# One-2-3-45/One-2-3-45

Hardware: AMD Instinct MI355X
Metric: rays/sec + mesh-extract wall-clock per scene (8x256^2 views, 128^3 vol) (higher is better)
Workload: dtype f32 (matrix products as 3 f16 MFMAs on split operands, fp32 accumulate); 1 GPU; BASELINE config 2: 1 scene/GPU/step (a different seeded scene every step), 8 views 256x256, 128^3 volume, 262144 rays (64+64 samples), mesh grid 256^3; whole scene pass per step; views=8, volume=128, rays=262144, mesh_res=256, parallelism=scenes x1, precision=f16x3

## Files before the change

### one-2-3-45_amd/csrc/color_net.h

```cpp
#pragma once
#include "common.h"
#include "geom_math.h"
#include "split_f16.h"

namespace o2345 {

#define MFMA32(a, b, c) __builtin_amdgcn_mfma_f32_32x32x2f32((a), (b), (c), 0, 0, 0)

constexpr int CM_A_RD0 = 0;
constexpr int CM_A_RD1 = CM_A_RD0 + 1 * 2 * 64;
constexpr int CM_A_B0 = CM_A_RD1 + 2 * 8 * 64;
constexpr int CM_A_B1 = CM_A_B0 + 2 * 32 * 64;
constexpr int CM_A_V0 = CM_A_B1 + 32 * 64;
constexpr int CM_A_V1 = CM_A_V0 + 16 * 64;
constexpr int CM_A_V20 = CM_A_V1 + 16 * 64;
constexpr int CM_A_R0 = CM_A_V20 + 16 * 64;
constexpr int CM_A_R1 = CM_A_R0 + 19 * 64;
constexpr int CM_BIAS0 = CM_A_R1 + 8 * 64;
constexpr int CM_B_RD0 = CM_BIAS0, CM_B_RD1 = CM_B_RD0 + 32, CM_B_B0 = CM_B_RD1 + 64, CM_B_B1 = CM_B_B0 + 64,
              CM_B_V0 = CM_B_B1 + 32, CM_B_V1 = CM_B_V0 + 32, CM_B_V20 = CM_B_V1 + 32, CM_B_R0 = CM_B_V20 + 32,
              CM_B_R1 = CM_B_R0 + 32, CM_V_V1X = CM_B_R1 + 32, CM_V_V21 = CM_V_V1X + 32, CM_V_R2 = CM_V_V21 + 32;
constexpr int CM_W_S = CM_V_R2 + 32;
constexpr int CM_S = CM_W_S + 144 * 64;
constexpr int CM_TOTAL = CM_S + 4;
constexpr int CX_A_RD0 = 0;
constexpr int CX_A_RD1 = CX_A_RD0 + 1 * 1 * 512;
constexpr int CX_A_B0 = CX_A_RD1 + 2 * 1 * 512;
constexpr int CX_A_B1 = CX_A_B0 + 2 * 4 * 512;
constexpr int CX_A_V0 = CX_A_B1 + 4 * 512;
constexpr int CX_A_V1 = CX_A_V0 + 2 * 512;
constexpr int CX_A_V20 = CX_A_V1 + 2 * 512;
constexpr int CX_A_R0 = CX_A_V20 + 2 * 512;
constexpr int CX_A_R1 = CX_A_R0 + 3 * 512;
constexpr int CX_A_END = CX_A_R1 + 1 * 512;
constexpr int CX_TOTAL = CX_A_END + (CM_TOTAL - CM_BIAS0);
constexpr int CM_A_S = CM_TOTAL;
constexpr int CM_TOTAL2 = CM_A_S + 2 * 72 * 64;
constexpr int CX_A_S = CX_TOTAL;
constexpr int CX_TOTAL2 = CX_A_S + 2 * 9 * 512;

struct ColorMArgs {
    const float* blob;
    const float* vol_cl; const float* maskvol; int D;
    const float* cmaps; const float* proj; const float* cam_pos; int V, H, W_img;
    const float* pts; const int* index; const int* n_dev; long long n;
    const float* query_cam; const float* normals;
    float* out_rgb; uint8_t* out_nviews;
    const float* f_geo;
    const float* f_rgb;
    const float* f_rdiff;
    const float* f_mask;
    unsigned long long* stats;
    int sched;
};

inline int color_sched_mode() { return knobs().color_sched; }
#if defined(__HIPCC__)
__device__ __forceinline__ void set_wave_prio(int p) {
    switch (p) {
        case 0: __builtin_amdgcn_s_setprio(0); break;
        case 1: __builtin_amdgcn_s_setprio(1); break;
        case 2: __builtin_amdgcn_s_setprio(2); break;
        default: __builtin_amdgcn_s_setprio(3); break;
    }
}
#endif

constexpr float LOG2E = 1.44269504088896340736f, LN2 = 0.69314718055994530942f;
__device__ __forceinline__ float celu(float y) {
    const float t = __builtin_amdgcn_fmed3f(__builtin_amdgcn_exp2f(y), 0.f, 1.f);
    return fmaxf(y, fmaf(t, LOG2E, -LOG2E));
}
typedef float f32x2 __attribute__((ext_vector_type(2)));
__device__ __forceinline__ f32x2 celu2(float y0, float y1) {
    f32x2 t;
    t[0] = __builtin_amdgcn_fmed3f(__builtin_amdgcn_exp2f(y0), 0.f, 1.f);
    t[1] = __builtin_amdgcn_fmed3f(__builtin_amdgcn_exp2f(y1), 0.f, 1.f);
    const f32x2 e = __builtin_elementwise_fma(t, f32x2{LOG2E, LOG2E}, f32x2{-LOG2E, -LOG2E});
    return f32x2{fmaxf(y0, e[0]), fmaxf(y1, e[1])};
}
__device__ __forceinline__ float crcp(float x) { return __builtin_amdgcn_rcpf(x); }
__device__ __forceinline__ float csigm(float z) { return crcp(1.f + __builtin_amdgcn_exp2f(-z)); }

template <int NB, int NST, int N>
__device__ __forceinline__ void cm_run(f32x16 (&acc)[NB], const float* A , int step0, const float (&b)[N]) {
    float cur[NB], nxt[NB];
#pragma unroll
    for (int nb = 0; nb < NB; ++nb) cur[nb] = A[(nb * NST + step0) * 64];
#pragma unroll
    for (int r = 0; r < N; ++r) {
        if (r + 1 < N) {
#pragma unroll
            for (int nb = 0; nb < NB; ++nb) nxt[nb] = A[(nb * NST + step0 + r + 1) * 64];
        }
#pragma unroll
        for (int nb = 0; nb < NB; ++nb) acc[nb] = MFMA32(cur[nb], b[r], acc[nb]);
#pragma unroll
        for (int nb = 0; nb < NB; ++nb) cur[nb] = nxt[nb];
        __builtin_amdgcn_sched_barrier(0);
    }
}

template <int NB, int N>
__device__ __forceinline__ void cx_run(f32x16 (&acc)[NB], const float4* A , const float (&b)[N], float m1) {
    constexpr int NS = (N + 7) / 8;
#pragma unroll
    for (int s = 0; s < NS; ++s) {
        const Split8 sp = split8(b, 8 * s, m1);
        h16x8 ahi[NB], alo[NB];
#pragma unroll
        for (int nb = 0; nb < NB; ++nb) {
            ahi[nb] = __builtin_bit_cast(h16x8, A[((nb * NS + s) * 2 + 0) * 64]);
            alo[nb] = __builtin_bit_cast(h16x8, A[((nb * NS + s) * 2 + 1) * 64]);
        }
#pragma unroll
        for (int nb = 0; nb < NB; ++nb) acc[nb] = MFMA_F16(alo[nb], sp.hi, acc[nb]);
#pragma unroll
        for (int nb = 0; nb < NB; ++nb) acc[nb] = MFMA_F16(ahi[nb], sp.lo, acc[nb]);
#pragma unroll
        for (int nb = 0; nb < NB; ++nb) acc[nb] = MFMA_F16(ahi[nb], sp.hi, acc[nb]);
        __builtin_amdgcn_sched_barrier(0);
    }
}
template <int NB, int N>
__device__ __forceinline__ void cx_run_from(f32x16 (&acc)[NB], const f32x16 (&init)[NB], const float4* A, const float (&b)[N], float m1) {
    constexpr int NS = (N + 7) / 8;
#pragma unroll
    for (int s = 0; s < NS; ++s) {
        const Split8 sp = split8(b, 8 * s, m1);
        h16x8 ahi[NB], alo[NB];
#pragma unroll
        for (int nb = 0; nb < NB; ++nb) {
            ahi[nb] = __builtin_bit_cast(h16x8, A[((nb * NS + s) * 2 + 0) * 64]);
            alo[nb] = __builtin_bit_cast(h16x8, A[((nb * NS + s) * 2 + 1) * 64]);
        }
#pragma unroll
        for (int nb = 0; nb < NB; ++nb) acc[nb] = MFMA_F16(alo[nb], sp.hi, s == 0 ? init[nb] : acc[nb]);
#pragma unroll
        for (int nb = 0; nb < NB; ++nb) acc[nb] = MFMA_F16(ahi[nb], sp.lo, acc[nb]);
#pragma unroll
        for (int nb = 0; nb < NB; ++nb) acc[nb] = MFMA_F16(ahi[nb], sp.hi, acc[nb]);
        __builtin_amdgcn_sched_barrier(0);
    }
}
template <bool X3, int NB, int N>
__device__ __forceinline__ void cm_layer(f32x16 (&acc)[NB], const float* lds, int lane, int off32, int offx, const float (&b)[N], float m1) {
    if constexpr (X3) cx_run<NB, N>(acc, reinterpret_cast<const float4*>(lds + offx) + lane, b, m1);
    else cm_run<NB, N, N>(acc, lds + lane + off32, 0, b);
}

template <int NB>
__device__ __forceinline__ void cm_bias(f32x16 (&acc)[NB], const float* bias, int h) {
#pragma unroll
    for (int nb = 0; nb < NB; ++nb) {
        const float4* p = reinterpret_cast<const float4*>(bias + (nb * 2 + h) * 16);
#pragma unroll
        for (int q = 0; q < 4; ++q) {
            const float4 t = p[q];
            acc[nb][4 * q] = t.x; acc[nb][4 * q + 1] = t.y; acc[nb][4 * q + 2] = t.z; acc[nb][4 * q + 3] = t.w;
        }
    }
}

template <int CTRL>
__device__ __forceinline__ float dpp_mov(float v) {
    return __builtin_bit_cast(float, __builtin_amdgcn_update_dpp(0, __builtin_bit_cast(int, v), CTRL, 0xf, 0xf, true));
}
#define O2345_GROUP_REDUCE(NAME, OP)                                                   \
    template <int G>                                                                   \
    __device__ __forceinline__ float NAME(float v) {                                   \
        v = OP(v, dpp_mov<0xB1>(v));                          \
        v = OP(v, dpp_mov<0x4E>(v));                          \
        if (G >= 8) v = OP(v, dpp_mov<0x141>(v));             \
        if (G >= 16) v = OP(v, dpp_mov<0x140>(v));            \
        if (G >= 32) v = OP(v, __shfl_xor(v, 16));                                     \
        return v;                                                                      \
    }
__device__ __forceinline__ float op_add(float a, float b) { return a + b; }
O2345_GROUP_REDUCE(gsum, op_add)
O2345_GROUP_REDUCE(gmin, fminf)
O2345_GROUP_REDUCE(gmax, fmaxf)
#undef O2345_GROUP_REDUCE

__device__ __forceinline__ void cm_project(const float* __restrict__ P, float x, float y, float z, int H, int W, float& gx, float& gy) {
    const float X = P[0] * x + P[1] * y + P[2] * z + P[3];
    const float Y = P[4] * x + P[5] * y + P[6] * z + P[7];
    const float Z = fmaxf(P[8] * x + P[9] * y + P[10] * z + P[11], 1e-3f);
    const float rz = crcp(Z), rw = crcp((float)(W - 1)), rh = crcp((float)(H - 1));
    auto div = [](float a_, float b_, float r_) { const float q = a_ * r_; return fmaf(fmaf(-b_, q, a_), r_, q); };
    gx = div(2.f * div(X, Z, rz), (float)(W - 1), rw) - 1.f;
    gy = div(2.f * div(Y, Z, rz), (float)(H - 1), rh) - 1.f;
    if (gx > 1.f || gx < -1.f) gx = 2.f;
    if (gy > 1.f || gy < -1.f) gy = 2.f;
}


#if defined(__HIPCC__)
struct ViewGeom {
    float rd[4];
    float e;
    float m;
    float gx, gy;
};

__device__ __forceinline__ ViewGeom view_geom(const ColorMArgs& a, int v, float px, float py, float pz, float qx, float qy, float qz,
                                              bool gvalid, float s_abs) {
    ViewGeom g;
    cm_project(a.proj + 12 * v, px, py, pz, a.H, a.W_img, g.gx, g.gy);
    g.m = (gvalid && fabsf(g.gx) < 1.f && fabsf(g.gy) < 1.f) ? 1.f : 0.f;
    const float sx = a.cam_pos[3 * v] - px, sy = a.cam_pos[3 * v + 1] - py, sz = a.cam_pos[3 * v + 2] - pz;
    const float rsn = crcp(sqrtf(sx * sx + sy * sy + sz * sz) + 1e-6f);
    const float ux = sx * rsn, uy = sy * rsn, uz = sz * rsn;
    const float dx = qx - ux, dy = qy - uy, dz = qz - uz;
    const float rdn = crcp(fmaxf(sqrtf(dx * dx + dy * dy + dz * dz), 1e-6f));
    g.rd[0] = dx * rdn; g.rd[1] = dy * rdn; g.rd[2] = dz * rdn;
    g.rd[3] = qx * ux + qy * uy + qz * uz;
    g.e = __builtin_amdgcn_exp2f(s_abs * (g.rd[3] - 1.f));
    return g;
}

#endif

int project_features_launch(const float* vol_cl, const float* maskvol, int D, const float* cmaps, const float* proj, const float* cam_pos, int V, int H, int W,
                            const float* pts, long long n, const float* query_cam, const float* normals, float* geo, float* rgb_feat, float* rdiff, float* mask,
                            void* stream);
int color_feats_launch(int x3, const float* blob, const float* geo, const float* rgb_feat, const float* ray_diff, const float* mask, int V, long long n,
                       float* out_rgb, uint8_t* out_nviews, void* stream);
int color_pts_launch(int x3, const float* blob, const float* vol_cl, const float* maskvol, int D, const float* cmaps, const float* proj,
                     const float* cam_pos, int V, int H, int W, const float* pts, const int32_t* index, const int32_t* n_dev, long long n,
                     const float* query_cam, const float* normals, float* out_rgb, uint8_t* out_nviews, unsigned long long* stats_dev, void* stream);

}
```

### one-2-3-45_amd/csrc/color_pts.hip

```cpp
#include "color_net.h"

namespace o2345 {

__device__ __forceinline__ void gather_now(const ColorMArgs& a, int h, int v, const ViewGeom& g, float (&rf)[32]) {
#pragma unroll
    for (int c = 0; c < 32; ++c) rf[c] = 0.f;
    const Taps2D tp = bilinear_taps(g.gx, g.gy, a.H, a.W_img);
    const float4* img = reinterpret_cast<const float4*>(a.cmaps + (size_t)v * a.H * a.W_img * 64) + 8 * h;
#pragma unroll
    for (int k = 0; k < 4; ++k)
        if (tp.w[k] != 0.f) {
            const float4* px4 = img + (size_t)tp.idx[k] * 16;
            const float wk = tp.w[k] * LOG2E;
#pragma unroll
            for (int q = 0; q < 8; ++q) {
                const float4 t = px4[q];
                rf[4 * q] = fmaf(t.x, wk, rf[4 * q]); rf[4 * q + 1] = fmaf(t.y, wk, rf[4 * q + 1]);
                rf[4 * q + 2] = fmaf(t.z, wk, rf[4 * q + 2]); rf[4 * q + 3] = fmaf(t.w, wk, rf[4 * q + 3]);
            }
        }
}

__device__ __forceinline__ ViewGeom feat_geom(const ColorMArgs& a, int v, long long slot, float s_abs) {
    ViewGeom g;
    const float4 rd = *reinterpret_cast<const float4*>(a.f_rdiff + ((size_t)v * a.n + slot) * 4);
    g.rd[0] = rd.x; g.rd[1] = rd.y; g.rd[2] = rd.z; g.rd[3] = rd.w;
    g.e = __builtin_amdgcn_exp2f(s_abs * (rd.w - 1.f));
    g.m = a.f_mask[(size_t)v * a.n + slot] != 0.f ? 1.f : 0.f;
    g.gx = g.gy = 0.f;
    return g;
}
__device__ __forceinline__ void load_feats(const ColorMArgs& a, int h, int v, long long slot, float (&rf)[32]) {
    const float* src = a.f_rgb + ((size_t)v * a.n + slot) * 59 + 32 * h;
#pragma unroll
    for (int c = 0; c < 32; ++c) rf[c] = (h == 0 || c < 27) ? src[(h == 0 || c < 27) ? c : 0] * LOG2E : 0.f;
}

template <bool X3>
__device__ __forceinline__ void direction_layer1(const float* lds, int tail, int lane, int h, const ViewGeom& g, float m1, float (&d16)[8]) {
    f32x16 acc1[1];
    cm_bias<1>(acc1, lds + tail + CM_B_RD0, h);
    const float b0[2] = {h ? g.rd[1] : g.rd[0], h ? g.rd[3] : g.rd[2]};
    cm_layer<X3, 1, 2>(acc1, lds, lane, CM_A_RD0, CX_A_RD0, b0, m1);
#pragma unroll
    for (int r = 0; r < 8; r += 2) { const f32x2 e2 = celu2(acc1[0][r], acc1[0][r + 1]); d16[r] = e2[0]; d16[r + 1] = e2[1]; }
}
template <bool X3>
__device__ __forceinline__ void direction_layer2(const float* lds, int tail, int lane, int h, const float (&d16)[8], float m1, float (&rf)[32]) {
    f32x16 acc2[2];
    cm_bias<2>(acc2, lds + tail + CM_B_RD1, h);
    cm_layer<X3, 2, 8>(acc2, lds, lane, CM_A_RD1, CX_A_RD1, d16, m1);
#pragma unroll
    for (int b = 0; b < 2; ++b)
#pragma unroll
        for (int r = 0; r < 16; r += 2) { const f32x2 e2 = celu2(acc2[b][r], acc2[b][r + 1]); rf[16 * b + r] += e2[0]; rf[16 * b + r + 1] += e2[1]; }
}

constexpr int CP_THREADS = 512;
template <bool X3, bool FEATS>
__global__ __launch_bounds__(CP_THREADS) void k_color_pts(ColorMArgs a) {
    extern __shared__ __attribute__((aligned(16))) float lds[];
    constexpr int HEAD = X3 ? (CX_A_END + CM_W_S - CM_BIAS0) : CM_W_S;
    constexpr int SRC_S = X3 ? (CX_TOTAL - 4) : CM_S;
    constexpr int NAS = X3 ? 2 * 9 * 512 : 2 * 72 * 64;
    constexpr int TAIL = X3 ? CX_A_END - CM_BIAS0 : 0;
    constexpr int L_S = HEAD, L_AS = HEAD + 4;
    for (int i = threadIdx.x * 4; i < HEAD; i += blockDim.x * 4)
        *reinterpret_cast<float4*>(lds + i) = *reinterpret_cast<const float4*>(a.blob + i);
    for (int i = threadIdx.x * 4; i < 4 + NAS; i += blockDim.x * 4)
        *reinterpret_cast<float4*>(lds + L_S + i) = *reinterpret_cast<const float4*>(a.blob + SRC_S + i);
    __syncthreads();
    const int lane = threadIdx.x & 63, j = lane & 31, h = lane >> 5;
    const int wave = threadIdx.x >> 6, nwave = blockDim.x >> 6;
    const long long n = a.n_dev ? (long long)*a.n_dev : a.n;
    const float m1 = X3 ? opaque_minus_one() : -1.f;
    const float s_abs = fabsf(lds[L_S]) * LOG2E;
    const int V = a.V;
    const bool skip_views = V <= 64 && !(a.sched & 4);
    const int base_prio = (a.sched & 1) ? (wave >> 2) : 0;
    if (a.sched & 1) set_wave_prio(base_prio);
    const TileSched ts = (a.sched & 8) ? TileSched{(long long)blockIdx.x * nwave + wave, (n + 31) / 32, (long long)gridDim.x * nwave}
                                       : tile_schedule(n, 32, wave, nwave);
    unsigned st_a = 0, st_b = 0, st_t = 0, st_full = 0;
    for (long long tile = ts.first; tile < ts.end; tile += ts.stride) {
        const long long i = tile * 32 + j;
        const bool live = i < n;
        const long long slot = live ? (a.index ? (long long)a.index[i] : i) : 0;
        const float px = (live && !FEATS) ? a.pts[3 * slot] : 0.f, py = (live && !FEATS) ? a.pts[3 * slot + 1] : 0.f,
                    pz = (live && !FEATS) ? a.pts[3 * slot + 2] : 0.f;
        float bs[72];
        bool gvalid;
        if constexpr (FEATS) {
            const float4* g4 = reinterpret_cast<const float4*>(a.f_geo + (size_t)slot * 16) + 2 * h;
            const float4 t0 = g4[0], t1 = g4[1];
            bs[0] = t0.x; bs[1] = t0.y; bs[2] = t0.z; bs[3] = t0.w; bs[4] = t1.x; bs[5] = t1.y; bs[6] = t1.z; bs[7] = t1.w;
            gvalid = true;
        } else {
#pragma unroll
            for (int c = 0; c < 8; ++c) bs[c] = 0.f;
            float msum = 0.f;
            const Axis2 ax = axis_taps_zeros(px, a.D), ay = axis_taps_zeros(py, a.D), az = axis_taps_zeros(pz, a.D);
#pragma unroll
            for (int tap = 0; tap < 8; ++tap) {
                const int ia = (tap >> 2) & 1, ib = (tap >> 1) & 1, ic = tap & 1;
                const float w = ax.w[ia] * ay.w[ib] * az.w[ic];
                if (w != 0.f) {
                    const size_t vox = ((size_t)ax.i[ia] * a.D + ay.i[ib]) * a.D + az.i[ic];
                    msum += w * a.maskvol[vox];
                    const float4* p4 = reinterpret_cast<const float4*>(a.vol_cl + vox * 16) + 2 * h;
#pragma unroll
                    for (int q = 0; q < 2; ++q) {
                        const float4 t = p4[q];
                        bs[4 * q] = fmaf(t.x, w, bs[4 * q]); bs[4 * q + 1] = fmaf(t.y, w, bs[4 * q + 1]);
                        bs[4 * q + 2] = fmaf(t.z, w, bs[4 * q + 2]); bs[4 * q + 3] = fmaf(t.w, w, bs[4 * q + 3]);
                    }
                }
            }
            gvalid = fabsf(px) < 1.f && fabsf(py) < 1.f && fabsf(pz) < 1.f && msum > 0.f;
        }
        float qx = 0.f, qy = 0.f, qz = 0.f;
        if constexpr (FEATS) {
        } else if (a.normals) {
            const float nx = a.normals[3 * slot], ny = a.normals[3 * slot + 1], nz = a.normals[3 * slot + 2];
            const float rn = crcp(fmaxf(sqrtf(nx * nx + ny * ny + nz * nz), 1e-6f));
            qx = nx * rn; qy = ny * rn; qz = nz * rn;
        } else {
            const float tx = a.query_cam[0] - px, ty = a.query_cam[1] - py, tz = a.query_cam[2] - pz;
            const float rn = crcp(sqrtf(tx * tx + ty * ty + tz * tz) + 1e-6f);
            qx = tx * rn; qy = ty * rn; qz = tz * rn;
        }
        float emin = INFINITY;
        for (int v = 0; v < V; ++v) {
            if constexpr (FEATS) {
                emin = fminf(emin, __builtin_amdgcn_exp2f(s_abs * (a.f_rdiff[((size_t)v * a.n + slot) * 4 + 3] - 1.f)));
                continue;
            }
            const float sx = a.cam_pos[3 * v] - px, sy = a.cam_pos[3 * v + 1] - py, sz = a.cam_pos[3 * v + 2] - pz;
            const float rsn = crcp(sqrtf(sx * sx + sy * sy + sz * sz) + 1e-6f);
            const float dot = qx * (sx * rsn) + qy * (sy * rsn) + qz * (sz * rsn);
            emin = fminf(emin, __builtin_amdgcn_exp2f(s_abs * (dot - 1.f)));
        }
        float wsum = 0.f, nvis = 0.f;
        unsigned long long active = 0ull;
        {
            float mean[32], m2[32];
#pragma unroll
            for (int c = 0; c < 32; ++c) { mean[c] = 0.f; m2[c] = 0.f; }
#pragma unroll 1
            for (int v = 0; v < V; ++v) {
                const ViewGeom g = FEATS ? feat_geom(a, v, slot, s_abs) : view_geom(a, v, px, py, pz, qx, qy, qz, gvalid, s_abs);
                if (skip_views && __builtin_amdgcn_ballot_w64(g.m != 0.f) == 0ull) continue;
                active |= 1ull << (v & 63);
                ++st_a;
                float rf[32];
                if constexpr (FEATS) load_feats(a, h, v, slot, rf);
                else {
                    if (a.sched & 2) set_wave_prio(3);
                    gather_now(a, h, v, g, rf);
                    if (a.sched & 2) set_wave_prio(base_prio);
                }
                {
                    float d16[8];
                    direction_layer1<X3>(lds, TAIL, lane, h, g, m1, d16);
                    direction_layer2<X3>(lds, TAIL, lane, h, d16, m1, rf);
                }
                const float raw = (g.e - emin) * g.m;
                nvis += g.m;
                wsum += raw;
                const float r0 = raw > 0.f ? raw * crcp(wsum) : 0.f;
                const float rq = raw > 0.f ? fmaf(fmaf(-wsum, r0, raw), crcp(wsum), r0) : 0.f;
#pragma unroll
                for (int c = 0; c < 32; ++c) {
                    const float d = rf[c] - mean[c];
                    mean[c] = fmaf(rq, d, mean[c]);
                    m2[c] = fmaf(raw * d, rf[c] - mean[c], m2[c]);
                }
            }
            const float rden = crcp(wsum + 1e-8f);
            const float S = wsum * rden, k2 = S * (1.f - S) * (1.f - S);
#pragma unroll
            for (int c = 0; c < 32; ++c) {
                bs[8 + c] = S * mean[c];
                bs[40 + c] = fmaf(k2 * mean[c], mean[c], m2[c] * rden);
            }
        }
        const float rden = crcp(wsum + 1e-8f);
        f32x16 sh[2];
        cm_bias<2>(sh, lds + TAIL + CM_B_B0, h);
        if constexpr (X3) cx_run<2, 72>(sh, reinterpret_cast<const float4*>(lds + L_AS) + lane, bs, m1);
        else cm_run<2, 72, 72>(sh, lds + L_AS + lane, 0, bs);
        float smax = -INFINITY, ssum = 0.f, o0 = 0.f, o1 = 0.f, o2 = 0.f;
        const bool skip_b = skip_views && __builtin_amdgcn_ballot_w64(live && nvis == 0.f) == 0ull;
        ++st_t;
        st_full += skip_b ? 0u : 1u;
#pragma unroll 1
        for (int v = 0; v < V; ++v) {
            if (skip_b && !((active >> (v & 63)) & 1ull)) continue;
            ++st_b;
            const ViewGeom g = FEATS ? feat_geom(a, v, slot, s_abs) : view_geom(a, v, px, py, pz, qx, qy, qz, gvalid, s_abs);
            const float m = g.m;
            float rf[32];
            if constexpr (FEATS) load_feats(a, h, v, slot, rf);
            else {
                if (a.sched & 2) set_wave_prio(3);
                gather_now(a, h, v, g, rf);
                if (a.sched & 2) set_wave_prio(base_prio);
            }
            const float rgb0 = rf[0], rgb1 = rf[1], rgb2 = rf[2];
            {
                float d16[8];
                direction_layer1<X3>(lds, TAIL, lane, h, g, m1, d16);
                direction_layer2<X3>(lds, TAIL, lane, h, d16, m1, rf);
            }
            const float wgt = (g.e - emin) * m * rden;
            f32x16 x32[1];
            {
                f32x16 acc[2];
                if constexpr (X3) cx_run_from<2, 32>(acc, sh, reinterpret_cast<const float4*>(lds + CX_A_B0) + lane, rf, m1);
                else { acc[0] = sh[0]; acc[1] = sh[1]; cm_layer<X3, 2, 32>(acc, lds, lane, CM_A_B0, CX_A_B0, rf, m1); }
                float hb[32];
#pragma unroll
                for (int b = 0; b < 2; ++b)
#pragma unroll
                    for (int r = 0; r < 16; r += 2) { const f32x2 e2 = celu2(acc[b][r], acc[b][r + 1]); hb[16 * b + r] = e2[0]; hb[16 * b + r + 1] = e2[1]; }
                cm_bias<1>(x32, lds + TAIL + CM_B_B1, h);
                cm_layer<X3, 1, 32>(x32, lds, lane, CM_A_B1, CX_A_B1, hb, m1);
#pragma unroll
                for (int r = 0; r < 16; r += 2) { const f32x2 e2 = celu2(x32[0][r], x32[0][r + 1]); x32[0][r] = e2[0]; x32[0][r + 1] = e2[1]; }
            }
            float vis;
            {
                float bin[16];
#pragma unroll
                for (int r = 0; r < 16; ++r) bin[r] = x32[0][r] * wgt;
                f32x16 t1[1];
                cm_bias<1>(t1, lds + TAIL + CM_B_V0, h);
                cm_layer<X3, 1, 16>(t1, lds, lane, CM_A_V0, CX_A_V0, bin, m1);
#pragma unroll
                for (int r = 0; r < 16; r += 2) { const f32x2 e2 = celu2(t1[0][r], t1[0][r + 1]); bin[r] = e2[0]; bin[r + 1] = e2[1]; }
                f32x16 t2[1];
                cm_bias<1>(t2, lds + TAIL + CM_B_V1, h);
                cm_layer<X3, 1, 16>(t2, lds, lane, CM_A_V1, CX_A_V1, bin, m1);
                float vr = 0.f;
#pragma unroll
                for (int r = 0; r < 16; ++r) vr = fmaf(bin[r], lds[TAIL + CM_V_V1X + h * 16 + r], vr);
                vr += __shfl_xor(vr, 32);
#pragma unroll
                for (int r = 0; r < 16; r += 2) { const f32x2 e2 = celu2(t2[0][r], t2[0][r + 1]); x32[0][r] += e2[0]; x32[0][r + 1] += e2[1]; }
                vis = csigm(celu(vr + lds[L_S + 1])) * m;
            }
            {
                float bin[16];
#pragma unroll
                for (int r = 0; r < 16; ++r) bin[r] = x32[0][r] * vis;
                f32x16 t1[1];
                cm_bias<1>(t1, lds + TAIL + CM_B_V20, h);
                cm_layer<X3, 1, 16>(t1, lds, lane, CM_A_V20, CX_A_V20, bin, m1);
#pragma unroll
                for (int r = 0; r < 16; r += 2) { const f32x2 e2 = celu2(t1[0][r], t1[0][r + 1]); bin[r] = e2[0]; bin[r + 1] = e2[1]; }
                float vr = 0.f;
#pragma unroll
                for (int r = 0; r < 16; ++r) vr = fmaf(bin[r], lds[TAIL + CM_V_V21 + h * 16 + r], vr);
                vr += __shfl_xor(vr, 32);
                vis = csigm(vr + lds[L_S + 2]) * m;
            }
            float score;
            {
                float bin[19];
#pragma unroll
                for (int r = 0; r < 16; ++r) bin[r] = x32[0][r];
                bin[16] = h ? g.rd[0] : vis; bin[17] = h ? g.rd[2] : g.rd[1]; bin[18] = h ? 0.f : g.rd[3];
                f32x16 t1[1];
                cm_bias<1>(t1, lds + TAIL + CM_B_R0, h);
                cm_layer<X3, 1, 19>(t1, lds, lane, CM_A_R0, CX_A_R0, bin, m1);
                float r16[8];
#pragma unroll
                for (int r = 0; r < 8; r += 2) { const f32x2 e2 = celu2(t1[0][r], t1[0][r + 1]); r16[r] = e2[0]; r16[r + 1] = e2[1]; }
                f32x16 t2[1];
                cm_bias<1>(t2, lds + TAIL + CM_B_R1, h);
                cm_layer<X3, 1, 8>(t2, lds, lane, CM_A_R1, CX_A_R1, r16, m1);
                float r8[4];
#pragma unroll
                for (int r = 0; r < 4; r += 2) { const f32x2 e2 = celu2(t2[0][r], t2[0][r + 1]); r8[r] = e2[0]; r8[r + 1] = e2[1]; }
                float sr = 0.f;
#pragma unroll
                for (int r = 0; r < 4; ++r) sr = fmaf(r8[r], lds[TAIL + CM_V_R2 + h * 16 + r], sr);
                score = sr + __shfl_xor(sr, 32) + lds[L_S + 3];
            }
            if (m == 0.f) score = -1e9f;
            const float nmax = fmaxf(smax, score);
            const float sc_old = __builtin_amdgcn_exp2f(smax - nmax), ex = __builtin_amdgcn_exp2f(score - nmax);
            ssum = fmaf(ssum, sc_old, ex);
            o0 = fmaf(o0, sc_old, ex * rgb0); o1 = fmaf(o1, sc_old, ex * rgb1); o2 = fmaf(o2, sc_old, ex * rgb2);
            smax = nmax;
        }
        if (live && h == 0) {
            const float rs = crcp(ssum) * LN2;
            a.out_rgb[3 * slot] = o0 * rs; a.out_rgb[3 * slot + 1] = o1 * rs; a.out_rgb[3 * slot + 2] = o2 * rs;
            if (a.out_nviews) a.out_nviews[slot] = (uint8_t)(nvis + 0.5f);
        }
    }
    if (a.stats && lane == 0) {
        atomicAdd(a.stats + 0, (unsigned long long)st_a); atomicAdd(a.stats + 1, (unsigned long long)st_b);
        atomicAdd(a.stats + 2, (unsigned long long)st_t); atomicAdd(a.stats + 3, (unsigned long long)st_full);
    }
}

}

namespace o2345 {

int color_pts_launch(int x3, const float* blob, const float* vol_cl, const float* maskvol, int D, const float* cmaps, const float* proj,
                           const float* cam_pos, int V, int H, int W, const float* pts, const int32_t* index, const int32_t* n_dev,
                           long long n, const float* query_cam, const float* normals, float* out_rgb, uint8_t* out_nviews,
                           unsigned long long* stats_dev , void* stream) {
    ColorMArgs a{blob, vol_cl, maskvol, D, cmaps, proj, cam_pos, V, H, W, pts, index, n_dev, n, query_cam, normals, out_rgb, out_nviews};
    a.sched = color_sched_mode();
    a.stats = stats_dev;
    const int n_cu = cu_count();
    const int threads = CP_THREADS;
    const long long per_block = (long long)(threads / 64) * 32;
    long long want = n_dev ? n_cu : (n + per_block - 1) / per_block;
    const unsigned grid = persistent_grid(want, n_cu);
    const size_t lds = (size_t)(x3 ? (CX_A_END + CM_W_S - CM_BIAS0) + 4 + 2 * 9 * 512 : CM_W_S + 4 + 2 * 72 * 64) * sizeof(float);
    hipStream_t s = (hipStream_t)stream;
    if (x3) {
        O2345_ENSURE_LDS((k_color_pts<true, false>), lds);
        hipLaunchKernelGGL((k_color_pts<true, false>), dim3(grid), dim3(threads), lds, s, a);
    } else {
        O2345_ENSURE_LDS((k_color_pts<false, false>), lds);
        hipLaunchKernelGGL((k_color_pts<false, false>), dim3(grid), dim3(threads), lds, s, a);
    }
    return check_launch("color_points (points-as-columns kernel)");
}

__global__ __launch_bounds__(256) void k_project_features(ColorMArgs a, float* __restrict__ geo , float* __restrict__ rgb_feat ,
                                                          float* __restrict__ rdiff , float* __restrict__ mask ) {
    const long long w = (long long)blockIdx.x * 4 + (threadIdx.x >> 6);
    if (w >= a.n * a.V) return;
    const long long p = w / a.V;
    const int v = (int)(w - p * a.V), c = threadIdx.x & 63;
    const float px = a.pts[3 * p], py = a.pts[3 * p + 1], pz = a.pts[3 * p + 2];
    float msum = 0.f, gch = 0.f;
    {
        const Axis2 ax = axis_taps_zeros(px, a.D), ay = axis_taps_zeros(py, a.D), az = axis_taps_zeros(pz, a.D);
#pragma unroll
        for (int tap = 0; tap < 8; ++tap) {
            const int ia = (tap >> 2) & 1, ib = (tap >> 1) & 1, ic = tap & 1;
            const float wt = ax.w[ia] * ay.w[ib] * az.w[ic];
            if (wt != 0.f) {
                const size_t vox = ((size_t)ax.i[ia] * a.D + ay.i[ib]) * a.D + az.i[ic];
                msum += wt * a.maskvol[vox];
                if (c < 16) gch = fmaf(a.vol_cl[vox * 16 + c], wt, gch);
            }
        }
    }
    const bool gvalid = fabsf(px) < 1.f && fabsf(py) < 1.f && fabsf(pz) < 1.f && msum > 0.f;
    float qx, qy, qz;
    if (a.normals) {
        const float nx = a.normals[3 * p], ny = a.normals[3 * p + 1], nz = a.normals[3 * p + 2];
        const float rn = crcp(fmaxf(sqrtf(nx * nx + ny * ny + nz * nz), 1e-6f));
        qx = nx * rn; qy = ny * rn; qz = nz * rn;
    } else {
        const float tx = a.query_cam[0] - px, ty = a.query_cam[1] - py, tz = a.query_cam[2] - pz;
        const float rn = crcp(sqrtf(tx * tx + ty * ty + tz * tz) + 1e-6f);
        qx = tx * rn; qy = ty * rn; qz = tz * rn;
    }
    const ViewGeom g = view_geom(a, v, px, py, pz, qx, qy, qz, gvalid, 0.f);
    float val = 0.f;
    {
        const Taps2D tp = bilinear_taps(g.gx, g.gy, a.H, a.W_img);
        const float* img = a.cmaps + (size_t)v * a.H * a.W_img * 64 + c;
#pragma unroll
        for (int k = 0; k < 4; ++k)
            if (tp.w[k] != 0.f) val = fmaf(img[(size_t)tp.idx[k] * 64], tp.w[k], val);
    }
    const size_t vp = (size_t)v * a.n + p;
    if (c < 59) rgb_feat[vp * 59 + c] = val;
    if (c < 4) rdiff[vp * 4 + c] = g.rd[c];
    if (c == 0) mask[vp] = g.m;
    if (v == 0 && c < 16) geo[(size_t)p * 16 + c] = gch;
}

int project_features_launch(const float* vol_cl, const float* maskvol, int D, const float* cmaps, const float* proj, const float* cam_pos, int V, int H, int W,
                            const float* pts, long long n, const float* query_cam, const float* normals, float* geo, float* rgb_feat, float* rdiff, float* mask,
                            void* stream) {
    ColorMArgs a{nullptr, vol_cl, maskvol, D, cmaps, proj, cam_pos, V, H, W, pts, nullptr, nullptr, n, query_cam, normals, nullptr, nullptr};
    hipLaunchKernelGGL(k_project_features, dim3(cdiv(n * V, 4)), dim3(256), 0, (hipStream_t)stream, a, geo, rgb_feat, rdiff, mask);
    return check_launch("project_features");
}

int color_feats_launch(int x3, const float* blob, const float* geo, const float* rgb_feat, const float* ray_diff, const float* mask, int V, long long n,
                       float* out_rgb, uint8_t* out_nviews, void* stream) {
    ColorMArgs a{};
    a.blob = blob; a.V = V; a.n = n; a.out_rgb = out_rgb; a.out_nviews = out_nviews;
    a.f_geo = geo; a.f_rgb = rgb_feat; a.f_rdiff = ray_diff; a.f_mask = mask;
    const int n_cu = cu_count();
    const long long per_block = (long long)(CP_THREADS / 64) * 32;
    const unsigned grid = persistent_grid((n + per_block - 1) / per_block, n_cu);
    const size_t lds = (size_t)(x3 ? (CX_A_END + CM_W_S - CM_BIAS0) + 4 + 2 * 9 * 512 : CM_W_S + 4 + 2 * 72 * 64) * sizeof(float);
    hipStream_t s = (hipStream_t)stream;
    if (x3) {
        O2345_ENSURE_LDS((k_color_pts<true, true>), lds);
        hipLaunchKernelGGL((k_color_pts<true, true>), dim3(grid), dim3(CP_THREADS), lds, s, a);
    } else {
        O2345_ENSURE_LDS((k_color_pts<false, true>), lds);
        hipLaunchKernelGGL((k_color_pts<false, true>), dim3(grid), dim3(CP_THREADS), lds, s, a);
    }
    return check_launch("color_from_features");
}

}

namespace o2345 {
int preload_color_pts() {
    hipFuncAttributes at;
    return (int)hipFuncGetAttributes(&at, (const void*)(k_project_features));
}
}
```

Measured before the change: 4.329 million rays/s.

## Stream aggregation weights from global, spill m2/sh to LDS, raise block to 768 threads

The 72-input aggregation layer weights are no longer staged in LDS. They are streamed from global memory through buffer loads, with the next slice prefetched one step ahead. The freed LDS now holds per-wave slots for the running m2 variance accumulators and the shared hidden state. This cuts register pressure and allows 768 threads per block, and views with all-zero weight are also skipped. The cost is more global/L2 weight traffic and extra LDS round-trips per view, and the zero-weight skip changes which views run the MLP.

```diff
diff --git a/one-2-3-45_amd/csrc/color_net.h b/one-2-3-45_amd/csrc/color_net.h
--- a/one-2-3-45_amd/csrc/color_net.h
+++ b/one-2-3-45_amd/csrc/color_net.h
@@ -122,27 +122,6 @@
         __builtin_amdgcn_sched_barrier(0);
     }
 }
-template <int NB, int N>
-__device__ __forceinline__ void cx_run_from(f32x16 (&acc)[NB], const f32x16 (&init)[NB], const float4* A, const float (&b)[N], float m1) {
-    constexpr int NS = (N + 7) / 8;
-#pragma unroll
-    for (int s = 0; s < NS; ++s) {
-        const Split8 sp = split8(b, 8 * s, m1);
-        h16x8 ahi[NB], alo[NB];
-#pragma unroll
-        for (int nb = 0; nb < NB; ++nb) {
-            ahi[nb] = __builtin_bit_cast(h16x8, A[((nb * NS + s) * 2 + 0) * 64]);
-            alo[nb] = __builtin_bit_cast(h16x8, A[((nb * NS + s) * 2 + 1) * 64]);
-        }
-#pragma unroll
-        for (int nb = 0; nb < NB; ++nb) acc[nb] = MFMA_F16(alo[nb], sp.hi, s == 0 ? init[nb] : acc[nb]);
-#pragma unroll
-        for (int nb = 0; nb < NB; ++nb) acc[nb] = MFMA_F16(ahi[nb], sp.lo, acc[nb]);
-#pragma unroll
-        for (int nb = 0; nb < NB; ++nb) acc[nb] = MFMA_F16(ahi[nb], sp.hi, acc[nb]);
-        __builtin_amdgcn_sched_barrier(0);
-    }
-}
 template <bool X3, int NB, int N>
 __device__ __forceinline__ void cm_layer(f32x16 (&acc)[NB], const float* lds, int lane, int off32, int offx, const float (&b)[N], float m1) {
     if constexpr (X3) cx_run<NB, N>(acc, reinterpret_cast<const float4*>(lds + offx) + lane, b, m1);
diff --git a/one-2-3-45_amd/csrc/color_pts.hip b/one-2-3-45_amd/csrc/color_pts.hip
--- a/one-2-3-45_amd/csrc/color_pts.hip
+++ b/one-2-3-45_amd/csrc/color_pts.hip
@@ -56,27 +56,94 @@
         for (int r = 0; r < 16; r += 2) { const f32x2 e2 = celu2(acc2[b][r], acc2[b][r + 1]); rf[16 * b + r] += e2[0]; rf[16 * b + r + 1] += e2[1]; }
 }
 
-constexpr int CP_THREADS = 512;
+constexpr int CP_AS_BYTES = 2 * 9 * 512 * 4;
+template <int NB, int N>
+__device__ __forceinline__ void cx_run_global(f32x16 (&acc)[NB], __amdgpu_buffer_rsrc_t rs, int lane, const float (&b)[N], float m1) {
+    constexpr int NS = (N + 7) / 8;
+    auto fetch = [&](int nb, int s, int k) { return __builtin_bit_cast(h16x8, __builtin_amdgcn_raw_buffer_load_b128(rs, lane * 16, ((nb * NS + s) * 2 + k) * 1024, 0)); };
+    h16x8 cur[NB][2], nxt[NB][2];
+#pragma unroll
+    for (int nb = 0; nb < NB; ++nb) { cur[nb][0] = fetch(nb, 0, 0); cur[nb][1] = fetch(nb, 0, 1); }
+#pragma unroll
+    for (int s = 0; s < NS; ++s) {
+        if (s + 1 < NS) {
+#pragma unroll
+            for (int nb = 0; nb < NB; ++nb) { nxt[nb][0] = fetch(nb, s + 1, 0); nxt[nb][1] = fetch(nb, s + 1, 1); }
+        }
+        const Split8 sp = split8(b, 8 * s, m1);
+#pragma unroll
+        for (int nb = 0; nb < NB; ++nb) acc[nb] = MFMA_F16(cur[nb][1], sp.hi, acc[nb]);
+#pragma unroll
+        for (int nb = 0; nb < NB; ++nb) acc[nb] = MFMA_F16(cur[nb][0], sp.lo, acc[nb]);
+#pragma unroll
+        for (int nb = 0; nb < NB; ++nb) acc[nb] = MFMA_F16(cur[nb][0], sp.hi, acc[nb]);
+#pragma unroll
+        for (int nb = 0; nb < NB; ++nb) { cur[nb][0] = nxt[nb][0]; cur[nb][1] = nxt[nb][1]; }
+        __builtin_amdgcn_sched_barrier(0);
+    }
+}
+template <int NB, int N>
+__device__ __forceinline__ void cm_run_global(f32x16 (&acc)[NB], __amdgpu_buffer_rsrc_t rs, int lane, const float (&b)[N]) {
+    auto fetch = [&](int nb, int r) { return __builtin_bit_cast(float, __builtin_amdgcn_raw_buffer_load_b32(rs, lane * 4, (nb * N + r) * 256, 0)); };
+    float cur[NB], nxt[NB];
+#pragma unroll
+    for (int nb = 0; nb < NB; ++nb) cur[nb] = fetch(nb, 0);
+#pragma unroll
+    for (int r = 0; r < N; ++r) {
+        if (r + 1 < N) {
+#pragma unroll
+            for (int nb = 0; nb < NB; ++nb) nxt[nb] = fetch(nb, r + 1);
+        }
+#pragma unroll
+        for (int nb = 0; nb < NB; ++nb) acc[nb] = MFMA32(cur[nb], b[r], acc[nb]);
+#pragma unroll
+        for (int nb = 0; nb < NB; ++nb) cur[nb] = nxt[nb];
+        __builtin_amdgcn_sched_barrier(0);
+    }
+}
+
+__device__ __forceinline__ void sh_store(float4* slot, const f32x16 (&sh)[2]) {
+#pragma unroll
+    for (int nb = 0; nb < 2; ++nb)
+#pragma unroll
+        for (int q = 0; q < 4; ++q) slot[(nb * 4 + q) * 64] = make_float4(sh[nb][4 * q], sh[nb][4 * q + 1], sh[nb][4 * q + 2], sh[nb][4 * q + 3]);
+}
+__device__ __forceinline__ void sh_load(f32x16 (&acc)[2], const float4* slot) {
+#pragma unroll
+    for (int nb = 0; nb < 2; ++nb)
+#pragma unroll
+        for (int q = 0; q < 4; ++q) {
+            const float4 t = slot[(nb * 4 + q) * 64];
+            acc[nb][4 * q] = t.x; acc[nb][4 * q + 1] = t.y; acc[nb][4 * q + 2] = t.z; acc[nb][4 * q + 3] = t.w;
+        }
+}
+
+constexpr int CP_THREADS = 768;
+constexpr int CP_SH_FLOATS = 2 * 16 * 64;
+constexpr size_t color_pts_lds_bytes(int x3) {
+    return (size_t)((x3 ? CX_A_END + CM_W_S - CM_BIAS0 : CM_W_S) + 4 + (CP_THREADS / 64) * CP_SH_FLOATS) * sizeof(float);
+}
+static_assert(color_pts_lds_bytes(1) <= 160 * 1024 && color_pts_lds_bytes(0) <= 160 * 1024, "k_color_pts: LDS of a CU exceeded");
 template <bool X3, bool FEATS>
 __global__ __launch_bounds__(CP_THREADS) void k_color_pts(ColorMArgs a) {
     extern __shared__ __attribute__((aligned(16))) float lds[];
     constexpr int HEAD = X3 ? (CX_A_END + CM_W_S - CM_BIAS0) : CM_W_S;
     constexpr int SRC_S = X3 ? (CX_TOTAL - 4) : CM_S;
-    constexpr int NAS = X3 ? 2 * 9 * 512 : 2 * 72 * 64;
     constexpr int TAIL = X3 ? CX_A_END - CM_BIAS0 : 0;
-    constexpr int L_S = HEAD, L_AS = HEAD + 4;
+    constexpr int L_S = HEAD, L_SH = HEAD + 4;
     for (int i = threadIdx.x * 4; i < HEAD; i += blockDim.x * 4)
         *reinterpret_cast<float4*>(lds + i) = *reinterpret_cast<const float4*>(a.blob + i);
-    for (int i = threadIdx.x * 4; i < 4 + NAS; i += blockDim.x * 4)
-        *reinterpret_cast<float4*>(lds + L_S + i) = *reinterpret_cast<const float4*>(a.blob + SRC_S + i);
+    if (threadIdx.x == 0) *reinterpret_cast<float4*>(lds + L_S) = *reinterpret_cast<const float4*>(a.blob + SRC_S);
     __syncthreads();
     const int lane = threadIdx.x & 63, j = lane & 31, h = lane >> 5;
     const int wave = threadIdx.x >> 6, nwave = blockDim.x >> 6;
+    float4* const sh_slot = reinterpret_cast<float4*>(lds + L_SH + wave * CP_SH_FLOATS) + lane;
     const long long n = a.n_dev ? (long long)*a.n_dev : a.n;
     const float m1 = X3 ? opaque_minus_one() : -1.f;
     const float s_abs = fabsf(lds[L_S]) * LOG2E;
     const int V = a.V;
     const bool skip_views = V <= 64 && !(a.sched & 4);
+    const bool skip_zero = skip_views && !(a.sched & 16);
     const int base_prio = (a.sched & 1) ? (wave >> 2) : 0;
     if (a.sched & 1) set_wave_prio(base_prio);
     const TileSched ts = (a.sched & 8) ? TileSched{(long long)blockIdx.x * nwave + wave, (n + 31) / 32, (long long)gridDim.x * nwave}
@@ -143,14 +210,19 @@
         float wsum = 0.f, nvis = 0.f;
         unsigned long long active = 0ull;
         {
-            float mean[32], m2[32];
-#pragma unroll
-            for (int c = 0; c < 32; ++c) { mean[c] = 0.f; m2[c] = 0.f; }
+            float mean[32];
+#pragma unroll
+            for (int c = 0; c < 32; ++c) mean[c] = 0.f;
+            bool fresh = true;
 #pragma unroll 1
             for (int v = 0; v < V; ++v) {
+                asm volatile("" ::: "memory");
                 const ViewGeom g = FEATS ? feat_geom(a, v, slot, s_abs) : view_geom(a, v, px, py, pz, qx, qy, qz, gvalid, s_abs);
                 if (skip_views && __builtin_amdgcn_ballot_w64(g.m != 0.f) == 0ull) continue;
                 active |= 1ull << (v & 63);
+                const float raw = (g.e - emin) * g.m;
+                nvis += g.m;
+                if (skip_zero && __builtin_amdgcn_ballot_w64(live && raw != 0.f) == 0ull) continue;
                 ++st_a;
                 float rf[32];
                 if constexpr (FEATS) load_feats(a, h, v, slot, rf);
@@ -164,31 +236,48 @@
                     direction_layer1<X3>(lds, TAIL, lane, h, g, m1, d16);
                     direction_layer2<X3>(lds, TAIL, lane, h, d16, m1, rf);
                 }
-                const float raw = (g.e - emin) * g.m;
-                nvis += g.m;
                 wsum += raw;
                 const float r0 = raw > 0.f ? raw * crcp(wsum) : 0.f;
                 const float rq = raw > 0.f ? fmaf(fmaf(-wsum, r0, raw), crcp(wsum), r0) : 0.f;
 #pragma unroll
-                for (int c = 0; c < 32; ++c) {
-                    const float d = rf[c] - mean[c];
-                    mean[c] = fmaf(rq, d, mean[c]);
-                    m2[c] = fmaf(raw * d, rf[c] - mean[c], m2[c]);
+                for (int q = 0; q < 8; ++q) {
+                    float4 t = fresh ? make_float4(0.f, 0.f, 0.f, 0.f) : sh_slot[q * 64];
+                    float* m2 = reinterpret_cast<float*>(&t);
+#pragma unroll
+                    for (int k = 0; k < 4; ++k) {
+                        const int c = 4 * q + k;
+                        const float d = rf[c] - mean[c];
+                        mean[c] = fmaf(rq, d, mean[c]);
+                        m2[k] = fmaf(raw * d, rf[c] - mean[c], m2[k]);
+                    }
+                    sh_slot[q * 64] = t;
                 }
+                fresh = false;
             }
             const float rden = crcp(wsum + 1e-8f);
             const float S = wsum * rden, k2 = S * (1.f - S) * (1.f - S);
-#pragma unroll
-            for (int c = 0; c < 32; ++c) {
-                bs[8 + c] = S * mean[c];
-                bs[40 + c] = fmaf(k2 * mean[c], mean[c], m2[c] * rden);
+            asm volatile("" ::: "memory");
+#pragma unroll
+            for (int q = 0; q < 8; ++q) {
+                const float4 t = fresh ? make_float4(0.f, 0.f, 0.f, 0.f) : sh_slot[q * 64];
+                const float m2[4] = {t.x, t.y, t.z, t.w};
+#pragma unroll
+                for (int k = 0; k < 4; ++k) {
+                    const int c = 4 * q + k;
+                    bs[8 + c] = S * mean[c];
+                    bs[40 + c] = fmaf(k2 * mean[c], mean[c], m2[k] * rden);
+                }
             }
         }
         const float rden = crcp(wsum + 1e-8f);
-        f32x16 sh[2];
-        cm_bias<2>(sh, lds + TAIL + CM_B_B0, h);
-        if constexpr (X3) cx_run<2, 72>(sh, reinterpret_cast<const float4*>(lds + L_AS) + lane, bs, m1);
-        else cm_run<2, 72, 72>(sh, lds + L_AS + lane, 0, bs);
+        {
+            f32x16 sh[2];
+            cm_bias<2>(sh, lds + TAIL + CM_B_B0, h);
+            const __amdgpu_buffer_rsrc_t rs = __builtin_amdgcn_make_buffer_rsrc((void*)(a.blob + (X3 ? CX_A_S : CM_A_S)), 0, CP_AS_BYTES, 0x00020000);
+            if constexpr (X3) cx_run_global<2, 72>(sh, rs, lane, bs, m1);
+            else cm_run_global<2, 72>(sh, rs, lane, bs);
+            sh_store(sh_slot, sh);
+        }
         float smax = -INFINITY, ssum = 0.f, o0 = 0.f, o1 = 0.f, o2 = 0.f;
         const bool skip_b = skip_views && __builtin_amdgcn_ballot_w64(live && nvis == 0.f) == 0ull;
         ++st_t;
@@ -216,8 +305,8 @@
             f32x16 x32[1];
             {
                 f32x16 acc[2];
-                if constexpr (X3) cx_run_from<2, 32>(acc, sh, reinterpret_cast<const float4*>(lds + CX_A_B0) + lane, rf, m1);
-                else { acc[0] = sh[0]; acc[1] = sh[1]; cm_layer<X3, 2, 32>(acc, lds, lane, CM_A_B0, CX_A_B0, rf, m1); }
+                sh_load(acc, sh_slot);
+                cm_layer<X3, 2, 32>(acc, lds, lane, CM_A_B0, CX_A_B0, rf, m1);
                 float hb[32];
 #pragma unroll
                 for (int b = 0; b < 2; ++b)
@@ -322,7 +411,7 @@
     const long long per_block = (long long)(threads / 64) * 32;
     long long want = n_dev ? n_cu : (n + per_block - 1) / per_block;
     const unsigned grid = persistent_grid(want, n_cu);
-    const size_t lds = (size_t)(x3 ? (CX_A_END + CM_W_S - CM_BIAS0) + 4 + 2 * 9 * 512 : CM_W_S + 4 + 2 * 72 * 64) * sizeof(float);
+    const size_t lds = color_pts_lds_bytes(x3);
     hipStream_t s = (hipStream_t)stream;
     if (x3) {
         O2345_ENSURE_LDS((k_color_pts<true, false>), lds);
@@ -398,7 +487,7 @@
     const int n_cu = cu_count();
     const long long per_block = (long long)(CP_THREADS / 64) * 32;
     const unsigned grid = persistent_grid((n + per_block - 1) / per_block, n_cu);
-    const size_t lds = (size_t)(x3 ? (CX_A_END + CM_W_S - CM_BIAS0) + 4 + 2 * 9 * 512 : CM_W_S + 4 + 2 * 72 * 64) * sizeof(float);
+    const size_t lds = color_pts_lds_bytes(x3);
     hipStream_t s = (hipStream_t)stream;
     if (x3) {
         O2345_ENSURE_LDS((k_color_pts<true, true>), lds);
```

After: 4.512 million rays/s, median of 6. +4.2%, better.
